# antrea-io/theia

Measured on AMD Instinct MI355X. Metric: flow-records/sec, higher is better.
Workload: dtype u64 (aggregates) + f64 (detectors)

## Files before the change

theia_amd/_capi.py:

```python
import ctypes as C
import os

from . import build as _build

u64, i64, i32, u32, f64, f32 = C.c_uint64, C.c_int64, C.c_int32, C.c_uint32, C.c_double, C.c_float

TAD_ABI_VERSION = 13
TAD_KEY_SKIP = (1 << 64) - 1
TAD_OK = 0
TAD_ERR_INVALID_ARGUMENT, TAD_ERR_NO_DEVICE, TAD_ERR_OUT_OF_MEMORY, TAD_ERR_HIP = -1, -2, -3, -4
TAD_ERR_KEY_RANGE, TAD_ERR_GRID_TOO_LARGE, TAD_ERR_BUSY = -5, -6, -7
TAD_ALGO = {"EWMA": 0, "ARIMA": 1, "DBSCAN": 2, "DROP": 3}
TAD_AGG = {"": 0, None: 0, "None": 0, "pod": 1, "svc": 2, "external": 3}
TAD_OP = {"auto": 0, "max": 1, "sum": 2}
TAD_MEM_HOST, TAD_MEM_DEVICE = 0, 1
TAD_FLAG_EMIT_ALL_POINTS = 1
TAD_FLAG_KEY_U32, TAD_FLAG_TIME_U32 = 2, 4
TAD_KEY_SKIP32 = (1 << 32) - 1
TAD_FEATURE_NARROW_COLUMNS = 1
TAD_FEATURE_STREAM_DBSCAN = 2
TAD_STATE_HISTORY = 1


class Plan(C.Structure):
    _fields_ = [("stage0", i32), ("partition_pass", i32), ("histogram", i32), ("sparse", i32), ("sparse_classes", i32),
                ("ewma_emit", i32), ("ewma_emit_rows", u32), ("reserved0", i32), ("tile_cells", i32), ("sparse_sort", i32), ("reserved1", i32)]


PLAN_VALUES = {
    "stage0": {"auto": 0, "v1": 1, "v2": 2}, "partition_pass": {"auto": 0, "sort": 1, "wc": 2, "wc_sectors": 3}, "histogram": {"auto": 0, "exact": 1, "sampled": 2},
    "sparse": {"auto": 0, "never": 1, "always": 2}, "sparse_classes": {"auto": 0, "always": 1}, "ewma_emit": {"auto": 0, "staged": 0, "lane": 1}, "tile_cells": {"auto": 0, "wide": 1},
    "sparse_sort": {"auto": 0, "lsd": 1, "partition": 2},
}


def make_plan(**kw):
    p = Plan()
    for name, v in kw.items():
        if name not in dict((f[0], 1) for f in Plan._fields_):
            raise ValueError("unknown tad_plan field %r" % name)
        if isinstance(v, str):
            v = PLAN_VALUES[name][v]
        setattr(p, name, int(v))
    return p


class KeyColumns(C.Structure):
    _fields_ = [("n_rows", u64), ("n_cols", i32), ("cols_a", C.POINTER(C.c_void_p)), ("keep_a", C.c_void_p),
                ("cols_b", C.POINTER(C.c_void_p)), ("keep_b", C.c_void_p), ("memory", C.c_int)]


class StringColumn(C.Structure):
    _fields_ = [("n_rows", u64), ("offsets", C.c_void_p), ("offset_bits", i32), ("data", C.c_void_p), ("data_bytes", u64),
                ("validity", C.c_void_p), ("validity_offset", u64), ("memory", C.c_int)]


class EngineOpts(C.Structure):
    _fields_ = [("device", i32), ("stream", C.c_void_p), ("workspace_limit", u64), ("plan", Plan), ("max_jobs_in_flight", i32), ("reserved", i32)]


class Job(C.Structure):
    _fields_ = [("algo", C.c_int), ("agg_flow", C.c_int), ("value_op", C.c_int),
                ("start_time", i64), ("end_time", i64), ("ewma_alpha", f64), ("dbscan_eps", f64),
                ("dbscan_min_samples", i32), ("arima_maxiter", i32), ("drop_nsigma", f64), ("drop_min_samples", i32),
# ... 108 lines not shown
```

theia_amd/csrc/tad_capi.cpp:

```cpp
#include "tad_engine.h"

using namespace tad;
using namespace tadh;

namespace tadh {

int ensure_rcp_table(JobCtx *e, uint64_t T) {
  const uint64_t want = T + 2;
  if (want <= e->rcp_n) return TAD_OK;
  uint64_t cap = want < 1024 ? 1024 : want + want / 4;
  int rc = ensure(e, e->rcp_table, cap * sizeof(double));
  if (rc != TAD_OK) return rc;
  std::vector<double> h(cap);
  h[0] = 0.0;
  for (uint64_t i = 1; i < cap; ++i) h[i] = 1.0 / (double)i;
  HIP_TRY(e, hipMemcpyAsync(e->rcp_table.p, h.data(), cap * sizeof(double), hipMemcpyHostToDevice, e->stream));
  HIP_TRY(e, hipStreamSynchronize(e->stream));
  e->rcp_n = cap;
  return TAD_OK;
}

int ensure_key_buffers(JobCtx *e, uint64_t K) {
  int rc;
  const uint64_t k = K ? K : 1;
  if ((rc = ensure(e, e->sigma, k * sizeof(double))) != TAD_OK) return rc;
  if ((rc = ensure(e, e->n_pts, k * sizeof(uint32_t))) != TAD_OK) return rc;
  if ((rc = ensure(e, e->n_anom, k * sizeof(uint32_t))) != TAD_OK) return rc;
  if ((rc = ensure(e, e->off, (k + 1) * sizeof(unsigned long long))) != TAD_OK) return rc;
  if ((rc = ensure(e, e->scan_scratch, scan_scratch_elems(k) * sizeof(unsigned long long))) != TAD_OK) return rc;
  if ((rc = ensure(e, e->key_mean, k * sizeof(double))) != TAD_OK) return rc;
  if ((rc = ensure(e, e->key_m2, k * sizeof(double))) != TAD_OK) return rc;
  if ((rc = ensure(e, e->counters, kTailBytes)) != TAD_OK) return rc;
  return TAD_OK;
}

}

namespace {

int detect_and_count(JobCtx *e, Grid g, JobParams &jp, DevCounters *ctr, uint64_t *rows, bool stats_done = false) {
  hipStream_t s = e->stream;
  int rc;
  if ((rc = ensure_key_buffers(e, g.K)) != TAD_OK) return rc;
  if ((rc = ensure_rcp_table(e, g.T)) != TAD_OK) return rc;
  double *sigma = static_cast<double *>(e->sigma.p);
  uint32_t *n_pts = static_cast<uint32_t *>(e->n_pts.p);
  uint32_t *n_anom = static_cast<uint32_t *>(e->n_anom.p);
  unsigned long long *off = static_cast<unsigned long long *>(e->off.p);

  const bool ewma = jp.algo == TAD_ALGO_EWMA;
  const bool drop = jp.algo == TAD_ALGO_DROP;
  const bool db_fused = jp.algo == TAD_ALGO_DBSCAN && !jp.all_points && !stats_done && dbscan_uses_list(g);
  jp.lazy_sigma = db_fused;
  if (drop) {
    if ((rc = ensure(e, e->calc, (g.K * g.T ? g.K * g.T : 1) * sizeof(double))) != TAD_OK) return rc;
    launch_drop(s, g, jp.drop_nsigma, jp.drop_min_samples, static_cast<double *>(e->calc.p), sigma, n_pts,
                static_cast<double *>(e->key_mean.p), static_cast<double *>(e->key_m2.p), ctr);
  } else if (!stats_done && !db_fused)
    launch_key_sigma(s, g, jp.alpha, ewma && !jp.all_points, static_cast<const double *>(e->rcp_table.p), sigma, n_pts, n_anom, ctr, static_cast<double *>(e->key_mean.p),
                     static_cast<double *>(e->key_m2.p));
  if (jp.algo == TAD_ALGO_DBSCAN) {
    if ((rc = ensure(e, e->aux, dbscan_scratch_bytes(g))) != TAD_OK) return rc;
    if (dbscan_uses_list(g)) {
      DbscanStats dst{nullptr, nullptr, nullptr, nullptr};
      if (db_fused) dst = DbscanStats{n_pts, n_anom, static_cast<double *>(e->key_mean.p), static_cast<double *>(e->key_m2.p)};
      if (launch_dbscan(s, g, jp.eps, jp.min_samples, e->aux.p, dst, jp.settled && db_fused) != 0)
        return fail(e, TAD_ERR_HIP, "DBSCAN launch failed");
    } else {
      return fail(e, TAD_ERR_GRID_TOO_LARGE, "DBSCAN: series of %llu buckets are not supported", (unsigned long long)g.T);
    }
  } else if (jp.algo == TAD_ALGO_ARIMA) {
    if ((rc = ensure(e, e->calc, g.K * g.T * sizeof(double))) != TAD_OK) return rc;
    const size_t wsb = arima_workspace_bytes(g);
    if ((rc = ensure(e, e->aux, wsb)) != TAD_OK) return rc;
    const bool held = e->hold && e->hold->held;
    if (held) e->hold->release();
    const unsigned int *yielded_dev = nullptr;
    if (launch_arima(s, g, sigma, n_pts, jp.maxiter, static_cast<double *>(e->calc.p), ctr, e->aux.p, wsb, e->eng->pause_dev, &yielded_dev) != 0)
      return fail(e, TAD_ERR_HIP, "ARIMA launch failed");
    while (yielded_dev != nullptr && e->eng->pause_dev != nullptr) {
      unsigned int y = 0;
      HIP_TRY(e, hipMemcpyAsync(&y, yielded_dev, 4, hipMemcpyDeviceToHost, s));
      HIP_TRY(e, hipStreamSynchronize(s));
      if (y == 0) break;
      const auto t0 = std::chrono::steady_clock::now();
      while (__atomic_load_n(&e->eng->pause_count, __ATOMIC_ACQUIRE) != 0 && std::chrono::steady_clock::now() - t0 < std::chrono::milliseconds(2))
        std::this_thread::sleep_for(std::chrono::microseconds(50));
      const uint32_t grace = __atomic_load_n(&e->eng->pause_count, __ATOMIC_ACQUIRE) != 0 ? 24u : 0u;
      if (launch_arima_fit(s, g, sigma, n_pts, jp.maxiter, static_cast<double *>(e->calc.p), ctr, e->aux.p, e->eng->pause_dev, &yielded_dev, grace) != 0)
        return fail(e, TAD_ERR_HIP, "ARIMA launch failed");
      e->arima_relaunches++;
    }
    if (held) e->hold->acquire();
  }
  const uint32_t *cnt = n_anom;
  if (jp.all_points && jp.algo != TAD_ALGO_ARIMA && !drop) cnt = n_pts;
  else if (db_fused) {}
  else if (!ewma || jp.all_points) launch_count_flags(s, g, jp.all_points, n_anom);
  launch_scan_moments(s, cnt, off, g.K, static_cast<unsigned long long *>(e->scan_scratch.p), dev_total(e), n_pts,
                      static_cast<const double *>(e->key_mean.p), static_cast<const double *>(e->key_m2.p), dev_moments(e), db_fused ? ctr : nullptr);
  HIP_TRY(e, hipMemcpyAsync(e->tail_host, e->counters.p, kTailBytes, hipMemcpyDeviceToHost, s));
  HIP_TRY(e, hipStreamSynchronize(s));
  HIP_TRY(e, hipGetLastError());
  *rows = *e->total_host;
  return TAD_OK;
}

}

namespace tadh {

void emit_rows(JobCtx *e, Grid g, Lattice L, const JobParams &jp, OutRows out, uint64_t rows) {
  const int kind = jp.algo == TAD_ALGO_EWMA ? 0 : (jp.algo == TAD_ALGO_ARIMA ? 1 : (jp.algo == TAD_ALGO_DROP ? 3 : (jp.lazy_sigma ? 4 : 2)));
  if (kind == 4 && !jp.all_points &&
      launch_emit_dbscan_list(e->stream, g, L, e->aux.p, static_cast<const uint32_t *>(e->n_anom.p), static_cast<const unsigned long long *>(e->off.p), out))
    return;
  launch_emit(e->stream, g, L, kind, jp.all_points, jp.alpha, static_cast<const double *>(e->sigma.p),
              static_cast<const uint32_t *>(e->n_pts.p), static_cast<const double *>(kind == 3 ? e->key_mean.p : e->calc.p),
              static_cast<const unsigned long long *>(e->off.p), out, rows, e->plan.ewma_emit, e->plan.ewma_emit_rows);
}

}

namespace {

int make_result(JobCtx *e, uint64_t rows, bool with_anomaly, tad_mem out_memory, ResultPriv **out, OutRows *dev_rows,
                ResultBlock *dev_block) {
  ResultPriv *rp = new (std::nothrow) ResultPriv();
  if (!rp) return fail(e, TAD_ERR_OUT_OF_MEMORY, "out of host memory");
  memset(rp, 0, sizeof *rp);
  const size_t bytes = result_bytes(rows, with_anomaly);
  int rc = alloc_device_block(e, bytes, dev_block);
  if (rc != TAD_OK) { delete rp; return rc; }
  carve(dev_block->base, rows, with_anomaly, dev_rows);
  rp->pub.n_rows = rows;
  rp->pub.memory = out_memory;
  *out = rp;
  return TAD_OK;
}

int finish_result(JobCtx *e, ResultPriv *rp, uint64_t rows, bool with_anomaly, ResultBlock dev_block, OutRows dev_rows) {
  if (rp->pub.memory == TAD_MEM_DEVICE) {
    rp->block = dev_block.base;
    rp->block_cap = dev_block.cap;
    rp->pub.key_id = reinterpret_cast<uint64_t *>(dev_rows.key_id);
    rp->pub.flow_end_s = reinterpret_cast<int64_t *>(dev_rows.flow_end_s);
    rp->pub.throughput = dev_rows.throughput;
    rp->pub.algo_calc = dev_rows.algo_calc;
    rp->pub.stddev = dev_rows.stddev;
    rp->pub.anomaly = dev_rows.anomaly;
    return TAD_OK;
  }
// ... 1219 lines not shown
```

theia_amd/csrc/tad_engine.cpp:

```cpp
#include "tad_engine.h"

using namespace tad;
using namespace tadh;

namespace tadh {

thread_local std::string g_static_err;

bool plan_ok(const tad_plan &p) {
  return p.stage0 >= 0 && p.stage0 <= 2 && p.partition_pass >= 0 && p.partition_pass <= 3 && p.histogram >= 0 && p.histogram <= 2 && p.sparse >= 0 &&
         p.sparse <= 2 && p.sparse_classes >= 0 && p.sparse_classes <= 1 && p.ewma_emit >= 0 && p.ewma_emit <= 1 && p.ewma_emit_rows <= 4096 && p.tile_cells >= 0 && p.tile_cells <= 1 && p.sparse_sort >= 0 && p.sparse_sort <= 2 && p.reserved0 == 0 && p.reserved1 == 0;
}

int vfail(tad_engine *e, int code, const char *fmt, va_list ap) {
  char buf[512];
  vsnprintf(buf, sizeof buf, fmt, ap);
  if (e) {
    std::lock_guard<std::mutex> lk(e->err_mu);
    e->err = buf;
  } else {
    g_static_err = buf;
  }
  return code;
}
int fail(tad_engine *e, int code, const char *fmt, ...) {
  va_list ap;
  va_start(ap, fmt);
  const int rc = vfail(e, code, fmt, ap);
  va_end(ap);
  return rc;
}
int fail(JobCtx *c, int code, const char *fmt, ...) {
  va_list ap;
  va_start(ap, fmt);
  const int rc = vfail(c ? c->eng : nullptr, code, fmt, ap);
  va_end(ap);
  return rc;
}
int fail(std::nullptr_t, int code, const char *fmt, ...) {
  va_list ap;
  va_start(ap, fmt);
  const int rc = vfail(nullptr, code, fmt, ap);
  va_end(ap);
  return rc;
// ... 394 lines not shown
```

theia_amd/csrc/tad_engine.h:

```cpp
#ifndef THEIA_TAD_ENGINE_H
#define THEIA_TAD_ENGINE_H

#include <atomic>
#include <chrono>
#include <condition_variable>
#include <cstdarg>
#include <cstdio>
#include <cstdlib>
#include <cstring>
#include <mutex>
#include <new>
#include <string>
#include <thread>
#include <vector>

#include "tad_internal.h"

struct DevBuf {
  void *p = nullptr;
  size_t cap = 0;
};

struct FreeBlock {
  void *p;
// ... 20 lines not shown
  int pause_count = 0;
  int *pause_dev = nullptr;
  hipStream_t signal_stream = nullptr;
  std::mutex pool_mu;
  std::vector<FreeBlock> free_blocks;
};

struct PauseHold;
struct JobCtx {
  tad_engine *eng = nullptr;
  PauseHold *hold = nullptr;
  int index = 0;
  bool busy = false;
  int device = 0;
  hipStream_t stream = nullptr;
  hipStream_t stream_normal = nullptr, stream_low = nullptr;
  bool own_streams = false;
  uint64_t ws_limit = 0;
  tad_plan plan{};
  std::atomic<int32_t> done{0}, total{0};
  char id[64] = {};
  DevBuf grid_val, grid_flag, sigma, n_pts, n_anom, off, scan_scratch, calc, counters, meta, aux, key_mean, key_m2;
  DevBuf in_key, in_key2, in_te, in_ts, in_val;
  DevBuf rcp_table;
  uint64_t rcp_n = 0;
  DevBuf binhist, part_total, part_start, part_offs32, recs, ovf, slices;
  DevBuf sp_comp_a, sp_comp_b, sp_val_a, sp_val_b, sp_temp, sp_first, sp_times;
  DevBuf sp_cls;
  DevBuf hs_key, hs_t, hs_val, hs_sorted, hs_noise, hs_cnt, hs_row, hs_koff, hs_kcnt;
  int arima_relaunches = 0;
  bool sp_by_partition = false;
  DevBuf part_fin;
  DevBuf ovf_keys;
  hipEvent_t ev[8] = {};
  tad::MetaPartial *meta_host = nullptr;
  unsigned char *tail_host = nullptr;
  tad::DevCounters *ctr_host = nullptr;
  unsigned long long *total_host = nullptr;
  tad::Moments *moments_host = nullptr;
  struct Learnt {
    bool valid = false;
    uint64_t n = 0, K = 0;
    bool has2 = false;
    int algo = 0, op = 0;
    bool exact_hist = false;
    uint32_t exact_uses = 0, exact_backoff = 8;
    bool wide_tiles = false;
  } learnt;
};

struct tad_state {
  uint64_t K = 0;
  void *block[2] = {nullptr, nullptr};
  int cur = 0;
  bool history = false;
  unsigned long long *hist_off[2] = {nullptr, nullptr};
  unsigned long long *hist_val[2] = {nullptr, nullptr};
  uint64_t hist_cap[2] = {0, 0};
  uint64_t hist_len[2] = {0, 0};
  mutable std::mutex mu;
};

struct PauseHold {
  tad_engine *eng;
  bool held = false;
  explicit PauseHold(tad_engine *e) : eng(e) {}
// ... 18 lines not shown
using namespace tad;

extern thread_local std::string g_static_err;

constexpr size_t kTailCtr = 0, kTailTotal = 64, kTailOvfCount = 72, kTailHistLen = 80, kTailMoments = 128;
constexpr size_t kTailBytes = kTailMoments + sizeof(Moments) * kMomentBlocks;
inline unsigned long long *dev_total(JobCtx *e) { return reinterpret_cast<unsigned long long *>(static_cast<unsigned char *>(e->counters.p) + kTailTotal); }
inline unsigned long long *dev_ovf_count(JobCtx *e) { return reinterpret_cast<unsigned long long *>(static_cast<unsigned char *>(e->counters.p) + kTailOvfCount); }
inline Moments *dev_moments(JobCtx *e) { return reinterpret_cast<Moments *>(static_cast<unsigned char *>(e->counters.p) + kTailMoments); }

constexpr int kMetaBlocks = 2048;
constexpr int kSampleBlockShift = 7;
constexpr int kDefaultJobsInFlight = 4;
constexpr int kMaxJobsInFlight = 16;
constexpr uint32_t kOverflowCap = 1u << 20;

bool plan_ok(const tad_plan &p);
int fail(tad_engine *e, int code, const char *fmt, ...);
int fail(JobCtx *c, int code, const char *fmt, ...);
int fail(std::nullptr_t, int code, const char *fmt, ...);

#define HIP_TRY(e, call)                                                                         \
  do {                                                                                           \
    hipError_t err__ = (call);                                                                   \
    if (err__ != hipSuccess)                                                                     \
      return fail((e), err__ == hipErrorOutOfMemory ? TAD_ERR_OUT_OF_MEMORY : TAD_ERR_HIP,       \
                  "%s failed: %s (%s:%d)", #call, hipGetErrorString(err__), __FILE__, __LINE__); \
  } while (0)


template <typename F> void for_each_buf(JobCtx *c, F f) {
  DevBuf *bufs[] = {&c->grid_val, &c->grid_flag, &c->sigma, &c->n_pts, &c->n_anom, &c->off, &c->scan_scratch, &c->calc, &c->counters, &c->meta, &c->aux,
                    &c->key_mean, &c->key_m2, &c->rcp_table, &c->binhist, &c->part_total, &c->part_start, &c->part_offs32, &c->recs, &c->ovf, &c->slices,
                    &c->sp_comp_a, &c->sp_comp_b, &c->sp_val_a, &c->sp_val_b, &c->sp_temp, &c->sp_first, &c->sp_times, &c->sp_cls, &c->part_fin, &c->ovf_keys,
                    &c->in_key, &c->in_key2, &c->in_te, &c->in_ts, &c->in_val,
                    &c->hs_key, &c->hs_t, &c->hs_val, &c->hs_sorted, &c->hs_noise, &c->hs_cnt, &c->hs_row, &c->hs_koff, &c->hs_kcnt};
  for (DevBuf *b : bufs) f(*b);
}

void drop_buffers(JobCtx *c);
void trim_idle(tad_engine *eng, JobCtx *self);
int ensure(JobCtx *e, DevBuf &b, size_t bytes);
void preload_code_objects();
JobCtx *ctx_create(tad_engine *eng, bool first);
void ctx_destroy(JobCtx *c);

struct Lease {
  tad_engine *eng;
  JobCtx *c = nullptr;
  Lease(tad_engine *eng_, const char *id = nullptr, bool low_priority = false) : eng(eng_) {
    std::unique_lock<std::mutex> lk(eng->mu);
    for (;;) {
      for (JobCtx *x : eng->ctxs)
        if (!x->busy) { c = x; break; }
      if (c) break;
      if ((int)eng->ctxs.size() + eng->creating < eng->max_ctx) {
        ++eng->creating;
        lk.unlock();
        hipSetDevice(eng->device);
        JobCtx *n = ctx_create(eng, false);
        lk.lock();
        --eng->creating;
        if (n) { n->index = (int)eng->ctxs.size(); eng->ctxs.push_back(n); c = n; break; }
        if (eng->ctxs.empty()) return;
      }
      eng->cv.wait(lk);
    }
// ... 28 lines not shown
Lattice make_lattice(int64_t t0, int64_t step, uint64_t nb);
uint64_t host_gcd(uint64_t a, uint64_t b);

struct ResultBlock {
  void *base = nullptr;
  size_t cap = 0;
};

size_t result_bytes(uint64_t rows, bool with_anomaly);
void carve(void *base, uint64_t rows, bool with_anomaly, OutRows *o);
int alloc_device_block(JobCtx *e, size_t bytes, ResultBlock *rb);

struct ResultPriv {
  tad_result pub;
  void *block;
  size_t block_cap;
};

struct PointsPriv {
  tad_points pub;
  void *block;
  size_t block_cap;
};

struct JobParams {
  tad_algo algo;
  double alpha, eps;
  int min_samples, maxiter;
  double drop_nsigma;
  int drop_min_samples;
  bool all_points;
  bool lazy_sigma = false;
  bool settled = false;
};

int ensure_rcp_table(JobCtx *e, uint64_t T);
int ensure_key_buffers(JobCtx *e, uint64_t K);
void emit_rows(JobCtx *e, Grid g, Lattice L, const JobParams &jp, OutRows out, uint64_t rows = 0);

}

#endif
```

theia_amd/csrc/tad_internal.h:

```cpp
#pragma once
#include <hip/hip_runtime.h>
#include <stdint.h>
#include <type_traits>

#include "tad.h"

namespace tad {

struct Lattice {
  int64_t t0;
  int64_t step;
  uint64_t nb;
  uint64_t magic;
  int mode;
};

struct Grid {
  unsigned long long *val;
  uint8_t *flag;
  uint64_t K;
  uint64_t T;
  const long long *times;
};

// ... 144 lines not shown
  uint32_t f0, f1, f2;
  unsigned long long v0, v1, v2;
  load(0, f0, v0);
  load(1, f1, v1);
  for (uint64_t c = 0; c < nblk; ++c) {
    load(c + 2, f2, v2);
    const uint64_t t0 = c * 64;
    const double x0 = (double)v0;
    const unsigned long long present = __ballot((f0 & FLAG_PRESENT) != 0);
    block(c);
    int ord = 0;
    for (unsigned long long m = present; m; m &= m - 1, ++ord) {
      const int u = __ffsll((long long)m) - 1;
      step(t0 + (uint64_t)u, (uint8_t)readlane_u32(f0, u), readlane_f64(x0, u), ord);
    }
    f0 = f1; v0 = v1;
    f1 = f2; v1 = v2;
  }
}

__device__ __forceinline__ Moments chan_merge(Moments a, Moments b) {
  if (b.n == 0.0) return a;
  if (a.n == 0.0) return b;
  Moments r;
  r.n = a.n + b.n;
  const double d = b.mean - a.mean;
  r.mean = a.mean + d * (b.n / r.n);
  r.m2 = a.m2 + b.m2 + d * d * (a.n * b.n / r.n);
  return r;
}

#endif

void launch_key_sigma(hipStream_t s, Grid g, double alpha, bool ewma_count, const double *rcp, double *sigma,
                      uint32_t *n_pts, uint32_t *n_anom, DevCounters *ctr, double *key_mean, double *key_m2);
static constexpr int kMomentBlocks = 128;
void launch_moments(hipStream_t s, uint64_t K, const uint32_t *n_pts, const double *key_mean,
                    const double *key_m2, Moments *partials, DevCounters *ctr = nullptr);
void launch_count_flags(hipStream_t s, Grid g, bool all_points, uint32_t *n_anom);
void launch_scan(hipStream_t s, const uint32_t *cnt, unsigned long long *off, uint64_t K,
                 unsigned long long *scratch, unsigned long long *total_copy = nullptr);
size_t scan_scratch_elems(uint64_t K);
void launch_scan_moments(hipStream_t s, const uint32_t *cnt, unsigned long long *off, uint64_t K, unsigned long long *scratch,
                         unsigned long long *total_copy, const uint32_t *n_pts, const double *key_mean, const double *key_m2, Moments *partials,
                         DevCounters *ctr);
void launch_emit(hipStream_t s, Grid g, Lattice lat, int kind, bool all_points, double alpha,
                 const double *sigma, const uint32_t *n_pts, const double *calc,
                 const unsigned long long *off, OutRows out, uint64_t rows_hint = 0,
                 int ewma_emit = 0, uint32_t ewma_emit_rows = 0);
void launch_emit_points(hipStream_t s, Grid g, Lattice lat, const unsigned long long *off, unsigned long long *out_key,
                        long long *out_t, unsigned long long *out_val);
struct StreamState {
  uint32_t *n;
  double *avg, *m2, *ewma;
  long long *last_t;
  unsigned char *seen;
};
void launch_stream(hipStream_t s, Grid g, Lattice lat, double alpha, bool all_points, bool emit, StreamState cur, StreamState next,
                   uint32_t *n_anom, const unsigned long long *off, OutRows out, DevCounters *ctr);
void launch_stream_points(hipStream_t s, const unsigned long long *comp, const unsigned long long *val, const unsigned long long *poff, uint64_t K,
                          int64_t t0, double alpha, bool all_points, bool emit, StreamState cur, StreamState next, uint32_t *n_anom,
                          const unsigned long long *off, OutRows out, DevCounters *ctr);
void launch_hist_decode(hipStream_t s, const unsigned long long *comp, uint64_t P, int64_t t0, unsigned long long *nk, long long *nt);
void launch_hist_sort(hipStream_t s, const unsigned long long *nv, const unsigned long long *poff, uint64_t K, unsigned long long *ns,
                      uint32_t *long_list, unsigned int *long_count);
uint64_t hist_merge_chunks_bound(uint64_t K, uint64_t total_len);
void launch_hist_merge(hipStream_t s, uint64_t K, const unsigned long long *hoff_old, const unsigned long long *hval_old, const unsigned long long *poff,
                       const unsigned long long *ns, unsigned long long *hoff_new, unsigned long long *hval_new, uint32_t *chunks,
                       unsigned long long *coff, unsigned long long *scan_scratch, uint64_t chunks_bound);
void launch_hist_verdict(hipStream_t s, const unsigned long long *nk, const unsigned long long *nv, const unsigned long long *P_dev, uint64_t P_cap,
                         const unsigned long long *hoff, const unsigned long long *h, double eps, int min_samples, bool all_points, uint8_t *noise,
                         uint32_t *cnt);
void launch_hist_emit(hipStream_t s, const unsigned long long *nk, const long long *nt, const unsigned long long *nv, const unsigned long long *P_dev,
                      uint64_t P_cap, const uint8_t *noise, const uint32_t *cnt, const unsigned long long *row, StreamState next, bool all_points,
                      OutRows out);
void launch_ewma_values(hipStream_t s, Grid g, double alpha, double *calc);

struct DbscanStats {
  uint32_t *n_pts, *n_anom;
  double *key_mean, *key_m2;
};
struct SettleArgs {
// ... 154 lines not shown
```

theia_amd/csrc/tad_kernels.hip:

```cpp
#include <cstdlib>

#include "tad_internal.h"

namespace tad {

static constexpr int kBlock = 256;

__device__ __forceinline__ uint64_t gcd_u64(uint64_t a, uint64_t b) {
  if (a == 0) return b;
  if (b == 0) return a;
  if (((a | b) >> 32) == 0) {
    uint32_t x = (uint32_t)a, y = (uint32_t)b;
    while (y) { uint32_t r = x % y; x = y; y = r; }
    return x;
  }
  while (b) { uint64_t r = a % b; a = b; b = r; }
  return a;
}

__device__ __forceinline__ uint64_t absdiff_i64(int64_t a, int64_t b) {
  return a >= b ? (uint64_t)a - (uint64_t)b : (uint64_t)b - (uint64_t)a;
}

struct MetaAcc {
  int64_t tmin, tmax, tref;
  uint64_t g, used;
};

__device__ __forceinline__ MetaAcc meta_merge(MetaAcc a, const MetaAcc &b) {
  if (b.used == 0) return a;
  if (a.used == 0) return b;
  a.tmin = b.tmin < a.tmin ? b.tmin : a.tmin;
// ... 145 lines not shown
  }
  unsigned long long u = used;
  for (int d = 32; d >= 1; d >>= 1) {
    u += __shfl_down(u, d);
    err |= __shfl_down(err, d);
  }
  if ((threadIdx.x & 63) == 0) {
    if (u) atomicAdd(&ctr->rows_used, u);
    if (err) atomicOr(&ctr->err, err);
  }
}

void launch_scatter(hipStream_t s, const uint64_t *key, const uint64_t *key2, const int64_t *t_end,
                    const int64_t *t_start, const uint64_t *value, uint64_t n, RowFilter f,
                    Lattice lat, Grid g, bool op_max, DevCounters *ctr, int cw) {
  if (n == 0) return;
  auto aligned16 = [](const void *p) { return p == nullptr || (reinterpret_cast<uintptr_t>(p) & 15) == 0; };
  const bool vec = aligned16(key) && aligned16(key2) && aligned16(t_end) && aligned16(value) && n >= 2;
  const uint64_t work = vec ? (n >> 1) : n;
  int blocks = (int)((work + kBlock - 1) / kBlock);
  if (blocks > 256 * 16) blocks = 256 * 16;
  if (blocks < 1) blocks = 1;
  with_widths(cw, [&](auto k32, auto t32) {
#define TAD_LAUNCH_SCATTER(OPMAX, VEC) \
  hipLaunchKernelGGL((k_scatter<OPMAX, VEC, k32(), t32()>), dim3(blocks), dim3(kBlock), 0, s, key, key2, t_end, t_start, value, n, f, lat, g, ctr)
    if (op_max) { if (vec) TAD_LAUNCH_SCATTER(true, true); else TAD_LAUNCH_SCATTER(true, false); }
    else        { if (vec) TAD_LAUNCH_SCATTER(false, true); else TAD_LAUNCH_SCATTER(false, false); }
#undef TAD_LAUNCH_SCATTER
  });
}

static constexpr int kUnroll = 16;

template <bool EWMA_COUNT, bool RCP_LDS, bool COOP = false>
__global__ __launch_bounds__(kBlock) void k_key_sigma(Grid g, double alpha, const double *__restrict__ rcp_g, double *__restrict__ sigma,
                                                      uint32_t *__restrict__ n_pts,
                                                      uint32_t *__restrict__ n_anom, DevCounters *ctr,
                                                      double *__restrict__ key_mean, double *__restrict__ key_m2) {
  const uint64_t gtid = (uint64_t)blockIdx.x * kBlock + threadIdx.x;
  const uint64_t k = COOP ? gtid >> 6 : gtid;
  const bool writer = !COOP || (threadIdx.x & 63) == 0;
  extern __shared__ __attribute__((aligned(16))) unsigned char smem_rcp[];
  const double *rcp = rcp_g;
  if (RCP_LDS) {
    double *l = reinterpret_cast<double *>(smem_rcp);
    for (uint64_t i = threadIdx.x; i <= g.T; i += kBlock) l[i] = rcp_g[i];
    __syncthreads();
    rcp = l;
  }
  unsigned long long my_pts = 0;
  unsigned my_key = 0;
  if (k < g.K) {
    double cnt = 0.0, avg = 0.0, m2 = 0.0;
    uint32_t n = 0;
    auto sigma_step = [&](uint64_t, uint8_t fl, unsigned long long raw) {
      if (fl & FLAG_PRESENT) {
        const double x = (double)raw;
        cnt = cnt + 1.0;
        n++;
        const double d = x - avg;
        const double dn = RCP_LDS ? div_by_count(d, cnt, rcp[n]) : d / cnt;
        avg = avg + dn;
        m2 = m2 + d * (d - dn);
      }
    };
    if (COOP) {
      double rl = 0.0;
      walk_series_coop(g, k,
                       [&](uint64_t) { rl = 1.0 / (double)(n + 1u + (threadIdx.x & 63u)); },
                       [&](uint64_t, uint8_t, double x, int ord) {
                         cnt = cnt + 1.0;
                         n++;
                         const double d = x - avg;
                         const double dn = div_by_count(d, cnt, readlane_f64(rl, ord));
                         avg = avg + dn;
                         m2 = m2 + d * (d - dn);
                       });
    } else {
      walk_series(g, k, sigma_step);
    }
    const bool has_sigma = n >= 2;
    const double sg = has_sigma ? sqrt(m2 / (cnt - 1.0)) : 0.0;
    if (writer) {
      sigma[k] = sg;
      n_pts[k] = n;
      if (key_mean != nullptr) { key_mean[k] = avg; key_m2[k] = m2; }
      my_pts = n;
      my_key = n > 0;
    }
    if (EWMA_COUNT) {
      uint32_t a = 0;
      if (has_sigma) {
        const double one_minus = 1.0 - alpha;
        double e = 0.0;
        auto ewma_step = [&](uint64_t, uint8_t fl, unsigned long long raw) {
          if (fl & FLAG_PRESENT) {
            const double x = (double)raw;
            e = one_minus * e + alpha * x;
            a += fabs(x - e) > sg ? 1u : 0u;
          }
        };
        if (COOP) walk_series_coop(g, k, [](uint64_t) {}, [&](uint64_t, uint8_t, double x, int) {
                    e = one_minus * e + alpha * x;
                    a += fabs(x - e) > sg ? 1u : 0u;
                  });
        else walk_series(g, k, ewma_step);
      }
      if (writer) n_anom[k] = a;
    }
  }
  for (int d = 32; d >= 1; d >>= 1) {
    my_pts += __shfl_down(my_pts, d);
    my_key += __shfl_down(my_key, d);
  }
  if ((threadIdx.x & 63) == 0 && my_key) {
    atomicAdd(&ctr->n_points, my_pts);
    atomicAdd(&ctr->n_keys, (unsigned long long)my_key);
  }
}

void launch_key_sigma(hipStream_t s, Grid g, double alpha, bool ewma_count, const double *rcp, double *sigma,
                      uint32_t *n_pts, uint32_t *n_anom, DevCounters *ctr, double *key_mean, double *key_m2) {
  if (g.K == 0) return;
  const size_t lds = (size_t)(g.T + 1) * 8;
  const bool in_lds = lds <= 32768;
  if (coop_shape(g)) {
    const int cblocks = (int)((g.K * 64 + kBlock - 1) / kBlock);
#define TAD_KSC(EC, RL) hipLaunchKernelGGL((k_key_sigma<EC, RL, true>), dim3(cblocks), dim3(kBlock), RL ? lds : 0, s, g, alpha, rcp, sigma, n_pts, n_anom, ctr, key_mean, key_m2)
    if (ewma_count) { if (in_lds) TAD_KSC(true, true); else TAD_KSC(true, false); }
    else { if (in_lds) TAD_KSC(false, true); else TAD_KSC(false, false); }
#undef TAD_KSC
    return;
  }
  const int blocks = (int)((g.K + kBlock - 1) / kBlock);
#define TAD_KS(EC, RL) hipLaunchKernelGGL((k_key_sigma<EC, RL>), dim3(blocks), dim3(kBlock), RL ? lds : 0, s, g, alpha, rcp, sigma, n_pts, n_anom, ctr, key_mean, key_m2)
  if (ewma_count) { if (in_lds) TAD_KS(true, true); else TAD_KS(true, false); }
  else { if (in_lds) TAD_KS(false, true); else TAD_KS(false, false); }
#undef TAD_KS
}


struct MomentsArgs {
  uint64_t K;
  const uint32_t *n_pts;
  const double *key_mean, *key_m2;
  Moments *partials;
  DevCounters *ctr;
};

__device__ __forceinline__ void moments_block(uint32_t mb, uint64_t K, const uint32_t *__restrict__ n_pts,
                                              const double *__restrict__ key_mean,
                                              const double *__restrict__ key_m2,
                                              Moments *__restrict__ partials, DevCounters *ctr) {
  Moments acc{0.0, 0.0, 0.0};
  unsigned long long pts = 0, keys = 0;
  const uint64_t stride = (uint64_t)kMomentBlocks * kBlock;
  constexpr int kMU = 8;
  for (uint64_t k = (uint64_t)mb * kBlock + threadIdx.x; k < K; k += stride * kMU) {
    uint32_t n[kMU];
    double mean[kMU], m2[kMU];
#pragma unroll
    for (int u = 0; u < kMU; ++u) {
      const uint64_t ku = k + (uint64_t)u * stride;
      const bool in = ku < K;
      n[u] = in ? n_pts[ku] : 0u;
      mean[u] = in ? key_mean[ku] : 0.0;
      m2[u] = in ? key_m2[ku] : 0.0;
    }
// ... 258 lines not shown
          const ulonglong2 kk = make_ulonglong2(k, k);
          reinterpret_cast<ulonglong2 *>(out.key_id + pos)[0] = kk;
          reinterpret_cast<ulonglong2 *>(out.key_id + pos)[1] = kk;
          reinterpret_cast<longlong2 *>(out.flow_end_s + pos)[0] = make_longlong2(bt[0], bt[1]);
          reinterpret_cast<longlong2 *>(out.flow_end_s + pos)[1] = make_longlong2(bt[2], bt[3]);
          reinterpret_cast<double2 *>(out.throughput + pos)[0] = make_double2(bx[0], bx[1]);
          reinterpret_cast<double2 *>(out.throughput + pos)[1] = make_double2(bx[2], bx[3]);
          reinterpret_cast<double2 *>(out.algo_calc + pos)[0] = make_double2(ba[0], ba[1]);
          reinterpret_cast<double2 *>(out.algo_calc + pos)[1] = make_double2(ba[2], ba[3]);
          if (!LAZY) {
            const double2 ss = make_double2(sg, sg);
            reinterpret_cast<double2 *>(out.stddev + pos)[0] = ss;
            reinterpret_cast<double2 *>(out.stddev + pos)[1] = ss;
          }
          if (ALL) *reinterpret_cast<uint32_t *>(out.anomaly + pos) = (uint32_t)bv[0] | ((uint32_t)bv[1] << 8) | ((uint32_t)bv[2] << 16) | ((uint32_t)bv[3] << 24);
          pos += 4;
          nb = 0;
        }
      }
    }
  };
  if (COOP) walk_series_coop(g, k, [](uint64_t) {}, [&](uint64_t t, uint8_t fl, double x, int) { point(t, fl, x); });
  else walk_series(g, k, [&](uint64_t t, uint8_t fl, unsigned long long raw) { if (fl & FLAG_PRESENT) point(t, fl, (double)raw); });
#pragma unroll
  for (int i = 0; i < 3; ++i)
    if (i < nb) write_row(pos + i, bt[i], bx[i], ba[i], ALL && bv[i] != 0);
  if (LAZY) {
    sg = has_sigma ? sqrt(s_m2 / (s_cnt - 1.0)) : 0.0;
    if (COOP) { for (unsigned long long at = first + (threadIdx.x & 63); at < end; at += 64) out.stddev[at] = sg; }
    else { for (unsigned long long at = first; at < end; ++at) out.stddev[at] = sg; }
  }
}

static constexpr int kStageMarkTBits = 26;
__global__ __launch_bounds__(64) void k_emit_staged(Grid g, Lattice L, double alpha, const double *__restrict__ sigma,
                                                    const uint32_t *__restrict__ n_pts,
                                                    const unsigned long long *__restrict__ off, OutRows out, uint32_t cap) {
  extern __shared__ __attribute__((aligned(16))) unsigned char smem_stage[];
  double *s_e = reinterpret_cast<double *>(smem_stage);
  double *s_sg = s_e + cap;
  uint32_t *s_m = reinterpret_cast<uint32_t *>(s_sg + 64);
  const uint32_t lane = threadIdx.x;
  const uint64_t k0 = (uint64_t)blockIdx.x * 64;
  const uint64_t k = k0 + lane;
  const uint64_t kend = k0 + 64 < g.K ? k0 + 64 : g.K;
  const unsigned long long base = off[k0];
  const unsigned long long total = off[kend] - base;
  if (total == 0) return;
  const bool live = k < g.K;
  unsigned long long pos = live ? off[k] - base : 0;
  const unsigned long long end = live ? off[k + 1] - base : 0;
  const double sg = live ? sigma[k] : 0.0;
  s_sg[lane] = sg;
  if (pos != end) {
    const double one_minus = 1.0 - alpha;
    double e = 0.0;
    walk_series(g, k, [&](uint64_t t, uint8_t fl, unsigned long long raw) {
      if (!(fl & FLAG_PRESENT)) return;
      const double x = (double)raw;
      e = one_minus * e + alpha * x;
      if (fabs(x - e) > sg && pos < end) {
        if (pos < cap) {
          s_e[pos] = e;
          s_m[pos] = (lane << kStageMarkTBits) | (uint32_t)t;
        } else {
          const unsigned long long at = base + pos;
          out.key_id[at] = k;
          out.flow_end_s[at] = g.times != nullptr ? g.times[t * g.K + k] : (long long)(L.t0 + (int64_t)t * L.step);
          out.throughput[at] = x;
          out.algo_calc[at] = e;
          out.stddev[at] = sg;
        }
        pos++;
      }
    });
  }
  __syncthreads();
  const unsigned long long staged = total < cap ? total : cap;
  for (unsigned long long r = lane; r < staged; r += 64) {
    const uint32_t m = s_m[r];
    const uint32_t ln = m >> kStageMarkTBits;
    const uint64_t t = m & ((1u << kStageMarkTBits) - 1u);
    const uint64_t cell = t * g.K + (k0 + ln);
    const unsigned long long at = base + r;
    out.key_id[at] = k0 + ln;
    out.flow_end_s[at] = g.times != nullptr ? g.times[cell] : (long long)(L.t0 + (int64_t)t * L.step);
    out.throughput[at] = (double)g.val[cell];
    out.algo_calc[at] = s_e[r];
    out.stddev[at] = s_sg[ln];
  }
}

static uint32_t emit_stage_rows(uint64_t K, uint64_t rows_hint, int ewma_emit, uint32_t ewma_emit_rows) {
  if (ewma_emit == 1) return 0;
  uint64_t cap = 1536;
  if (rows_hint != 0) {
    const uint64_t mean = (rows_hint * 64 + K - 1) / K;
    cap = mean + mean / 8 + 128;
  }
  if (ewma_emit_rows != 0) cap = ewma_emit_rows;
  cap = (cap + 63) & ~63ull;
  if (cap < 64) cap = 64;
  if (cap > 4096) cap = 4096;
  return (uint32_t)cap;
}

void launch_emit(hipStream_t s, Grid g, Lattice lat, int kind, bool all_points, double alpha,
                 const double *sigma, const uint32_t *n_pts, const double *calc,
                 const unsigned long long *off, OutRows out, uint64_t rows_hint, int ewma_emit, uint32_t ewma_emit_rows) {
  if (g.K == 0) return;
  if (coop_shape(g)) {
    const int cblocks = (int)((g.K * 64 + kBlock - 1) / kBlock);
#define TAD_LAUNCH_EMIT_C(KIND, ALL) \
  hipLaunchKernelGGL((k_emit<KIND, ALL, true>), dim3(cblocks), dim3(kBlock), 0, s, g, lat, alpha, sigma, n_pts, calc, off, out)
    if (all_points) {
      if (kind == 0) TAD_LAUNCH_EMIT_C(0, true); else if (kind == 1) TAD_LAUNCH_EMIT_C(1, true); else if (kind == 3) TAD_LAUNCH_EMIT_C(3, true); else TAD_LAUNCH_EMIT_C(2, true);
    } else {
      if (kind == 0) TAD_LAUNCH_EMIT_C(0, false); else if (kind == 1) TAD_LAUNCH_EMIT_C(1, false); else if (kind == 3) TAD_LAUNCH_EMIT_C(3, false);
      else if (kind == 4) TAD_LAUNCH_EMIT_C(4, false); else TAD_LAUNCH_EMIT_C(2, false);
    }
#undef TAD_LAUNCH_EMIT_C
    return;
  }
  if (kind == 0 && !all_points && g.T < (1ull << kStageMarkTBits)) {
    if (const uint32_t cap = emit_stage_rows(g.K, rows_hint, ewma_emit, ewma_emit_rows)) {
      const unsigned blocks64 = (unsigned)((g.K + 63) / 64);
      hipLaunchKernelGGL(k_emit_staged, dim3(blocks64), dim3(64), (size_t)cap * 12 + 64 * 8, s, g, lat, alpha, sigma, n_pts, off, out, cap);
      return;
    }
  }
  const int blocks = (int)((g.K + kBlock - 1) / kBlock);
#define TAD_LAUNCH_EMIT(KIND, ALL) \
  hipLaunchKernelGGL((k_emit<KIND, ALL>), dim3(blocks), dim3(kBlock), 0, s, g, lat, alpha, sigma, n_pts, calc, off, out)
  if (all_points) {
    if (kind == 0) TAD_LAUNCH_EMIT(0, true); else if (kind == 1) TAD_LAUNCH_EMIT(1, true); else if (kind == 3) TAD_LAUNCH_EMIT(3, true); else TAD_LAUNCH_EMIT(2, true);
  } else {
    if (kind == 0) TAD_LAUNCH_EMIT(0, false); else if (kind == 1) TAD_LAUNCH_EMIT(1, false); else if (kind == 3) TAD_LAUNCH_EMIT(3, false);
    else if (kind == 4) TAD_LAUNCH_EMIT(4, false); else TAD_LAUNCH_EMIT(2, false);
  }
#undef TAD_LAUNCH_EMIT
}

__global__ __launch_bounds__(kBlock) void k_emit_points(Grid g, Lattice L, const unsigned long long *__restrict__ off,
                                                        unsigned long long *__restrict__ out_key, long long *__restrict__ out_t,
                                                        unsigned long long *__restrict__ out_val) {
  const uint64_t k = (uint64_t)blockIdx.x * kBlock + threadIdx.x;
  if (k >= g.K) return;
  unsigned long long pos = off[k];
  const unsigned long long end = off[k + 1];
  auto step = [&](uint64_t t, uint8_t fl, unsigned long long raw) {
    if ((fl & FLAG_PRESENT) && pos < end) {
      out_key[pos] = k;
      out_t[pos] = g.times != nullptr ? g.times[t * g.K + k] : (long long)(L.t0 + (int64_t)t * L.step);
      out_val[pos] = raw;
      pos++;
    }
  };
  uint64_t t = 0;
  for (; t + kUnroll <= g.T && pos < end; t += kUnroll) {
    uint8_t fl[kUnroll];
// ... 190 lines not shown
```

Before: 78.01 billion.

## Stage EWMA anomaly rows during sigma pass so emit copies instead of recomputing

```diff
diff --git a/theia_amd/_capi.py b/theia_amd/_capi.py
--- a/theia_amd/_capi.py
+++ b/theia_amd/_capi.py
@@ -29,7 +29,7 @@
 
 PLAN_VALUES = {
     "stage0": {"auto": 0, "v1": 1, "v2": 2}, "partition_pass": {"auto": 0, "sort": 1, "wc": 2, "wc_sectors": 3}, "histogram": {"auto": 0, "exact": 1, "sampled": 2},
-    "sparse": {"auto": 0, "never": 1, "always": 2}, "sparse_classes": {"auto": 0, "always": 1}, "ewma_emit": {"auto": 0, "staged": 0, "lane": 1}, "tile_cells": {"auto": 0, "wide": 1},
+    "sparse": {"auto": 0, "never": 1, "always": 2}, "sparse_classes": {"auto": 0, "always": 1}, "ewma_emit": {"auto": 0, "staged": 0, "copy": 0, "lane": 1, "walk": 2}, "tile_cells": {"auto": 0, "wide": 1},
     "sparse_sort": {"auto": 0, "lsd": 1, "partition": 2},
 }
 
diff --git a/theia_amd/csrc/tad_capi.cpp b/theia_amd/csrc/tad_capi.cpp
--- a/theia_amd/csrc/tad_capi.cpp
+++ b/theia_amd/csrc/tad_capi.cpp
@@ -56,9 +56,17 @@
     if ((rc = ensure(e, e->calc, (g.K * g.T ? g.K * g.T : 1) * sizeof(double))) != TAD_OK) return rc;
     launch_drop(s, g, jp.drop_nsigma, jp.drop_min_samples, static_cast<double *>(e->calc.p), sigma, n_pts,
                 static_cast<double *>(e->key_mean.p), static_cast<double *>(e->key_m2.p), ctr);
-  } else if (!stats_done && !db_fused)
+  } else if (!stats_done && !db_fused) {
+    jp.ewma_stage = EwmaStage{nullptr, nullptr, nullptr, 0};
+    if (ewma && !jp.all_points) {
+      if (const uint32_t cap = ewma_stage_rows(g, e->plan.ewma_emit, e->plan.ewma_emit_rows)) {
+        if ((rc = ensure(e, e->ewma_stage, ewma_stage_bytes(g.K, cap))) != TAD_OK) return rc;
+        jp.ewma_stage = ewma_stage_carve(e->ewma_stage.p, g.K, cap);
+      }
+    }
     launch_key_sigma(s, g, jp.alpha, ewma && !jp.all_points, static_cast<const double *>(e->rcp_table.p), sigma, n_pts, n_anom, ctr, static_cast<double *>(e->key_mean.p),
-                     static_cast<double *>(e->key_m2.p));
+                     static_cast<double *>(e->key_m2.p), jp.ewma_stage);
+  }
   if (jp.algo == TAD_ALGO_DBSCAN) {
     if ((rc = ensure(e, e->aux, dbscan_scratch_bytes(g))) != TAD_OK) return rc;
     if (dbscan_uses_list(g)) {
@@ -117,7 +125,8 @@
     return;
   launch_emit(e->stream, g, L, kind, jp.all_points, jp.alpha, static_cast<const double *>(e->sigma.p),
               static_cast<const uint32_t *>(e->n_pts.p), static_cast<const double *>(kind == 3 ? e->key_mean.p : e->calc.p),
-              static_cast<const unsigned long long *>(e->off.p), out, rows, e->plan.ewma_emit, e->plan.ewma_emit_rows);
+              static_cast<const unsigned long long *>(e->off.p), out, rows, e->plan.ewma_emit, e->plan.ewma_emit_rows,
+              kind == 0 && !jp.all_points && jp.ewma_stage.cap != 0 ? &jp.ewma_stage : nullptr);
 }
 
 }
diff --git a/theia_amd/csrc/tad_engine.cpp b/theia_amd/csrc/tad_engine.cpp
--- a/theia_amd/csrc/tad_engine.cpp
+++ b/theia_amd/csrc/tad_engine.cpp
@@ -9,7 +9,7 @@
 
 bool plan_ok(const tad_plan &p) {
   return p.stage0 >= 0 && p.stage0 <= 2 && p.partition_pass >= 0 && p.partition_pass <= 3 && p.histogram >= 0 && p.histogram <= 2 && p.sparse >= 0 &&
-         p.sparse <= 2 && p.sparse_classes >= 0 && p.sparse_classes <= 1 && p.ewma_emit >= 0 && p.ewma_emit <= 1 && p.ewma_emit_rows <= 4096 && p.tile_cells >= 0 && p.tile_cells <= 1 && p.sparse_sort >= 0 && p.sparse_sort <= 2 && p.reserved0 == 0 && p.reserved1 == 0;
+         p.sparse <= 2 && p.sparse_classes >= 0 && p.sparse_classes <= 1 && p.ewma_emit >= 0 && p.ewma_emit <= 2 && p.ewma_emit_rows <= 4096 && p.tile_cells >= 0 && p.tile_cells <= 1 && p.sparse_sort >= 0 && p.sparse_sort <= 2 && p.reserved0 == 0 && p.reserved1 == 0;
 }
 
 int vfail(tad_engine *e, int code, const char *fmt, va_list ap) {
diff --git a/theia_amd/csrc/tad_engine.h b/theia_amd/csrc/tad_engine.h
--- a/theia_amd/csrc/tad_engine.h
+++ b/theia_amd/csrc/tad_engine.h
@@ -76,6 +76,7 @@
   bool sp_by_partition = false;
   DevBuf part_fin;
   DevBuf ovf_keys;
+  DevBuf ewma_stage;
   hipEvent_t ev[8] = {};
   tad::MetaPartial *meta_host = nullptr;
   unsigned char *tail_host = nullptr;
@@ -160,7 +161,7 @@
 template <typename F> void for_each_buf(JobCtx *c, F f) {
   DevBuf *bufs[] = {&c->grid_val, &c->grid_flag, &c->sigma, &c->n_pts, &c->n_anom, &c->off, &c->scan_scratch, &c->calc, &c->counters, &c->meta, &c->aux,
                     &c->key_mean, &c->key_m2, &c->rcp_table, &c->binhist, &c->part_total, &c->part_start, &c->part_offs32, &c->recs, &c->ovf, &c->slices,
-                    &c->sp_comp_a, &c->sp_comp_b, &c->sp_val_a, &c->sp_val_b, &c->sp_temp, &c->sp_first, &c->sp_times, &c->sp_cls, &c->part_fin, &c->ovf_keys,
+                    &c->sp_comp_a, &c->sp_comp_b, &c->sp_val_a, &c->sp_val_b, &c->sp_temp, &c->sp_first, &c->sp_times, &c->sp_cls, &c->part_fin, &c->ovf_keys, &c->ewma_stage,
                     &c->in_key, &c->in_key2, &c->in_te, &c->in_ts, &c->in_val,
                     &c->hs_key, &c->hs_t, &c->hs_val, &c->hs_sorted, &c->hs_noise, &c->hs_cnt, &c->hs_row, &c->hs_koff, &c->hs_kcnt};
   for (DevBuf *b : bufs) f(*b);
@@ -255,6 +256,7 @@
   bool all_points;
   bool lazy_sigma = false;
   bool settled = false;
+  tad::EwmaStage ewma_stage{nullptr, nullptr, nullptr, 0};
 };
 
 int ensure_rcp_table(JobCtx *e, uint64_t T);
diff --git a/theia_amd/csrc/tad_internal.h b/theia_amd/csrc/tad_internal.h
--- a/theia_amd/csrc/tad_internal.h
+++ b/theia_amd/csrc/tad_internal.h
@@ -200,8 +200,16 @@
 
 #endif
 
+struct EwmaStage {
+  double *e;
+  uint32_t *m, *n;
+  uint32_t cap;
+};
+uint32_t ewma_stage_rows(const Grid &g, int ewma_emit, uint32_t ewma_emit_rows);
+size_t ewma_stage_bytes(uint64_t K, uint32_t cap);
+EwmaStage ewma_stage_carve(void *p, uint64_t K, uint32_t cap);
 void launch_key_sigma(hipStream_t s, Grid g, double alpha, bool ewma_count, const double *rcp, double *sigma,
-                      uint32_t *n_pts, uint32_t *n_anom, DevCounters *ctr, double *key_mean, double *key_m2);
+                      uint32_t *n_pts, uint32_t *n_anom, DevCounters *ctr, double *key_mean, double *key_m2, EwmaStage st = EwmaStage{nullptr, nullptr, nullptr, 0});
 static constexpr int kMomentBlocks = 128;
 void launch_moments(hipStream_t s, uint64_t K, const uint32_t *n_pts, const double *key_mean,
                     const double *key_m2, Moments *partials, DevCounters *ctr = nullptr);
@@ -215,7 +223,8 @@
 void launch_emit(hipStream_t s, Grid g, Lattice lat, int kind, bool all_points, double alpha,
                  const double *sigma, const uint32_t *n_pts, const double *calc,
                  const unsigned long long *off, OutRows out, uint64_t rows_hint = 0,
-                 int ewma_emit = 0, uint32_t ewma_emit_rows = 0);
+                 int ewma_emit = 0, uint32_t ewma_emit_rows = 0,
+                 const EwmaStage *stage = nullptr);
 void launch_emit_points(hipStream_t s, Grid g, Lattice lat, const unsigned long long *off, unsigned long long *out_key,
                         long long *out_t, unsigned long long *out_val);
 struct StreamState {
diff --git a/theia_amd/csrc/tad_kernels.hip b/theia_amd/csrc/tad_kernels.hip
--- a/theia_amd/csrc/tad_kernels.hip
+++ b/theia_amd/csrc/tad_kernels.hip
@@ -1,3 +1,4 @@
+#include <algorithm>
 #include <cstdlib>
 
 #include "tad_internal.h"
@@ -209,22 +210,74 @@
 
 static constexpr int kUnroll = 16;
 
-template <bool EWMA_COUNT, bool RCP_LDS, bool COOP = false>
+static constexpr int kStageMarkTBits = 26;
+static constexpr int kStageRankShift = 13;
+static constexpr uint32_t kStageRankMask = ((1u << (kStageMarkTBits - kStageRankShift)) - 1u) << kStageRankShift;
+static constexpr uint32_t kStageOverflow = 0xFFFFFFFFu;
+static size_t ewma_stage_lds_bytes(uint32_t cap) { return (size_t)cap * 14 + 64 * 4; }
+
+__device__ __forceinline__ void ewma_stage_wave(uint32_t a, const EwmaStage &st, const double *s_e, const uint32_t *s_m, uint16_t *s_idx,
+                                                uint32_t *s_base) {
+  const uint32_t lane = threadIdx.x & 63u;
+  __syncthreads();
+  uint32_t incl = a;
+  for (int d = 1; d < 64; d <<= 1) {
+    const uint32_t y = __shfl_up(incl, d);
+    if (lane >= (uint32_t)d) incl += y;
+  }
+  const uint32_t total = __shfl(incl, 63);
+  const uint64_t w = blockIdx.x;
+  if (lane == 0) st.n[w] = total <= st.cap ? total : kStageOverflow;
+  if (total > st.cap) return;
+  s_base[lane] = incl - a;
+  __syncthreads();
+  constexpr int kU = 4;
+  for (uint32_t r0 = lane; r0 < total; r0 += 64 * kU) {
+    uint32_t m[kU];
+#pragma unroll
+    for (int u = 0; u < kU; ++u) m[u] = r0 + 64 * u < total ? s_m[r0 + 64 * u] : 0u;
+#pragma unroll
+    for (int u = 0; u < kU; ++u)
+      if (r0 + 64 * u < total) s_idx[s_base[m[u] >> kStageMarkTBits] + ((m[u] & kStageRankMask) >> kStageRankShift)] = (uint16_t)(r0 + 64 * u);
+  }
+  __syncthreads();
+  double *ge = st.e + w * st.cap;
+  uint32_t *gm = st.m + w * st.cap;
+  for (uint32_t r0 = lane; r0 < total; r0 += 64 * kU) {
+    uint32_t i[kU];
+#pragma unroll
+    for (int u = 0; u < kU; ++u) i[u] = r0 + 64 * u < total ? s_idx[r0 + 64 * u] : 0u;
+#pragma unroll
+    for (int u = 0; u < kU; ++u)
+      if (r0 + 64 * u < total) {
+        ge[r0 + 64 * u] = s_e[i[u]];
+        gm[r0 + 64 * u] = s_m[i[u]] & ~kStageRankMask;
+      }
+  }
+}
+
+template <bool EWMA_COUNT, bool RCP_LDS, bool COOP = false, bool STAGE = false>
 __global__ __launch_bounds__(kBlock) void k_key_sigma(Grid g, double alpha, const double *__restrict__ rcp_g, double *__restrict__ sigma,
                                                       uint32_t *__restrict__ n_pts,
                                                       uint32_t *__restrict__ n_anom, DevCounters *ctr,
-                                                      double *__restrict__ key_mean, double *__restrict__ key_m2) {
-  const uint64_t gtid = (uint64_t)blockIdx.x * kBlock + threadIdx.x;
+                                                      double *__restrict__ key_mean, double *__restrict__ key_m2, EwmaStage st) {
+  constexpr int BS = STAGE ? 64 : kBlock;
+  const uint64_t gtid = (uint64_t)blockIdx.x * BS + threadIdx.x;
   const uint64_t k = COOP ? gtid >> 6 : gtid;
   const bool writer = !COOP || (threadIdx.x & 63) == 0;
   extern __shared__ __attribute__((aligned(16))) unsigned char smem_rcp[];
   const double *rcp = rcp_g;
   if (RCP_LDS) {
     double *l = reinterpret_cast<double *>(smem_rcp);
-    for (uint64_t i = threadIdx.x; i <= g.T; i += kBlock) l[i] = rcp_g[i];
+    for (uint64_t i = threadIdx.x; i <= g.T; i += BS) l[i] = rcp_g[i];
     __syncthreads();
     rcp = l;
   }
+  double *s_e = reinterpret_cast<double *>(smem_rcp);
+  uint32_t *s_m = reinterpret_cast<uint32_t *>(s_e + (STAGE ? st.cap : 0));
+  uint16_t *s_idx = reinterpret_cast<uint16_t *>(s_m + (STAGE ? st.cap : 0));
+  uint32_t *s_base = reinterpret_cast<uint32_t *>(s_idx + (STAGE ? st.cap : 0));
+  uint32_t a = 0;
   unsigned long long my_pts = 0;
   unsigned my_key = 0;
   if (k < g.K) {
@@ -266,12 +319,28 @@
       my_key = n > 0;
     }
     if (EWMA_COUNT) {
-      uint32_t a = 0;
+      if (STAGE) __builtin_amdgcn_wave_barrier();
       if (has_sigma) {
         const double one_minus = 1.0 - alpha;
         double e = 0.0;
-        auto ewma_step = [&](uint64_t, uint8_t fl, unsigned long long raw) {
-          if (fl & FLAG_PRESENT) {
+        uint32_t cursor = 0;
+        auto ewma_step = [&](uint64_t t, uint8_t fl, unsigned long long raw) {
+          if constexpr (STAGE) {
+            bool hit = false;
+            if (fl & FLAG_PRESENT) {
+              const double x = (double)raw;
+              e = one_minus * e + alpha * x;
+              hit = fabs(x - e) > sg;
+            }
+            const unsigned long long b = __ballot(hit);
+            const uint32_t slot = cursor + __builtin_amdgcn_mbcnt_hi((uint32_t)(b >> 32), __builtin_amdgcn_mbcnt_lo((uint32_t)b, 0u));
+            if (hit && slot < st.cap) {
+              s_e[slot] = e;
+              s_m[slot] = ((threadIdx.x & 63u) << kStageMarkTBits) | (a << kStageRankShift) | (uint32_t)t;
+            }
+            cursor += (uint32_t)__popcll(b);
+            a += hit ? 1u : 0u;
+          } else if (fl & FLAG_PRESENT) {
             const double x = (double)raw;
             e = one_minus * e + alpha * x;
             a += fabs(x - e) > sg ? 1u : 0u;
@@ -286,6 +355,7 @@
       if (writer) n_anom[k] = a;
     }
   }
+  if constexpr (STAGE) ewma_stage_wave(a, st, s_e, s_m, s_idx, s_base);
   for (int d = 32; d >= 1; d >>= 1) {
     my_pts += __shfl_down(my_pts, d);
     my_key += __shfl_down(my_key, d);
@@ -297,20 +367,28 @@
 }
 
 void launch_key_sigma(hipStream_t s, Grid g, double alpha, bool ewma_count, const double *rcp, double *sigma,
-                      uint32_t *n_pts, uint32_t *n_anom, DevCounters *ctr, double *key_mean, double *key_m2) {
+                      uint32_t *n_pts, uint32_t *n_anom, DevCounters *ctr, double *key_mean, double *key_m2, EwmaStage st) {
   if (g.K == 0) return;
   const size_t lds = (size_t)(g.T + 1) * 8;
   const bool in_lds = lds <= 32768;
+  if (ewma_count && st.cap != 0) {
+    const size_t slds = std::max(in_lds ? lds : (size_t)0, ewma_stage_lds_bytes(st.cap));
+    const unsigned blocks64 = (unsigned)((g.K + 63) / 64);
+#define TAD_KSS(RL) hipLaunchKernelGGL((k_key_sigma<true, RL, false, true>), dim3(blocks64), dim3(64), slds, s, g, alpha, rcp, sigma, n_pts, n_anom, ctr, key_mean, key_m2, st)
+    if (in_lds) TAD_KSS(true); else TAD_KSS(false);
+#undef TAD_KSS
+    return;
+  }
   if (coop_shape(g)) {
     const int cblocks = (int)((g.K * 64 + kBlock - 1) / kBlock);
-#define TAD_KSC(EC, RL) hipLaunchKernelGGL((k_key_sigma<EC, RL, true>), dim3(cblocks), dim3(kBlock), RL ? lds : 0, s, g, alpha, rcp, sigma, n_pts, n_anom, ctr, key_mean, key_m2)
+#define TAD_KSC(EC, RL) hipLaunchKernelGGL((k_key_sigma<EC, RL, true>), dim3(cblocks), dim3(kBlock), RL ? lds : 0, s, g, alpha, rcp, sigma, n_pts, n_anom, ctr, key_mean, key_m2, st)
     if (ewma_count) { if (in_lds) TAD_KSC(true, true); else TAD_KSC(true, false); }
     else { if (in_lds) TAD_KSC(false, true); else TAD_KSC(false, false); }
 #undef TAD_KSC
     return;
   }
   const int blocks = (int)((g.K + kBlock - 1) / kBlock);
-#define TAD_KS(EC, RL) hipLaunchKernelGGL((k_key_sigma<EC, RL>), dim3(blocks), dim3(kBlock), RL ? lds : 0, s, g, alpha, rcp, sigma, n_pts, n_anom, ctr, key_mean, key_m2)
+#define TAD_KS(EC, RL) hipLaunchKernelGGL((k_key_sigma<EC, RL>), dim3(blocks), dim3(kBlock), RL ? lds : 0, s, g, alpha, rcp, sigma, n_pts, n_anom, ctr, key_mean, key_m2, st)
   if (ewma_count) { if (in_lds) TAD_KS(true, true); else TAD_KS(true, false); }
   else { if (in_lds) TAD_KS(false, true); else TAD_KS(false, false); }
 #undef TAD_KS
@@ -635,10 +713,8 @@
   }
 }
 
-static constexpr int kStageMarkTBits = 26;
-__global__ __launch_bounds__(64) void k_emit_staged(Grid g, Lattice L, double alpha, const double *__restrict__ sigma,
-                                                    const uint32_t *__restrict__ n_pts,
-                                                    const unsigned long long *__restrict__ off, OutRows out, uint32_t cap) {
+__device__ __forceinline__ void emit_staged_wave(Grid g, Lattice L, double alpha, const double *__restrict__ sigma,
+                                                 const unsigned long long *__restrict__ off, OutRows out, uint32_t cap) {
   extern __shared__ __attribute__((aligned(16))) unsigned char smem_stage[];
   double *s_e = reinterpret_cast<double *>(smem_stage);
   double *s_sg = s_e + cap;
@@ -694,6 +770,66 @@
   }
 }
 
+__global__ __launch_bounds__(64) void k_emit_staged(Grid g, Lattice L, double alpha, const double *__restrict__ sigma,
+                                                    const uint32_t *__restrict__ n_pts,
+                                                    const unsigned long long *__restrict__ off, OutRows out, uint32_t cap) {
+  emit_staged_wave(g, L, alpha, sigma, off, out, cap);
+}
+
+__global__ __launch_bounds__(64) void k_emit_copy(Grid g, Lattice L, double alpha, const double *__restrict__ sigma,
+                                                  const unsigned long long *__restrict__ off, OutRows out, uint32_t cap, EwmaStage st) {
+  extern __shared__ __attribute__((aligned(16))) unsigned char smem_stage[];
+  const uint32_t lane = threadIdx.x;
+  const uint64_t w = blockIdx.x;
+  const uint64_t k0 = w * 64;
+  const uint64_t kend = k0 + 64 < g.K ? k0 + 64 : g.K;
+  const unsigned long long base = off[k0];
+  const unsigned long long total = off[kend] - base;
+  if (total == 0) return;
+  if (st.n[w] != total) {
+    emit_staged_wave(g, L, alpha, sigma, off, out, cap);
+    return;
+  }
+  double *s_sg = reinterpret_cast<double *>(smem_stage);
+  s_sg[lane] = k0 + lane < g.K ? sigma[k0 + lane] : 0.0;
+  __syncthreads();
+  const double *__restrict__ ge = st.e + w * st.cap;
+  const uint32_t *__restrict__ gm = st.m + w * st.cap;
+  constexpr int kU = 8;
+  for (unsigned long long r0 = lane; r0 < total; r0 += 64 * kU) {
+    double e[kU];
+    uint32_t m[kU];
+    unsigned long long v[kU];
+    long long ts[kU];
+#pragma unroll
+    for (int u = 0; u < kU; ++u) {
+      const unsigned long long r = r0 + 64 * u;
+      e[u] = r < total ? ge[r] : 0.0;
+      m[u] = r < total ? gm[r] : 0u;
+    }
+#pragma unroll
+    for (int u = 0; u < kU; ++u) {
+      const uint64_t t = m[u] & ((1u << kStageMarkTBits) - 1u);
+      const uint64_t cell = t * g.K + (k0 + (m[u] >> kStageMarkTBits));
+      const bool in = r0 + 64 * u < total;
+      v[u] = in ? g.val[cell] : 0ull;
+      ts[u] = !in ? 0ll : (g.times != nullptr ? g.times[cell] : (long long)(L.t0 + (int64_t)t * L.step));
+    }
+#pragma unroll
+    for (int u = 0; u < kU; ++u) {
+      const unsigned long long r = r0 + 64 * u;
+      if (r < total) {
+        const unsigned long long at = base + r;
+        out.key_id[at] = k0 + (m[u] >> kStageMarkTBits);
+        out.flow_end_s[at] = ts[u];
+        out.throughput[at] = (double)v[u];
+        out.algo_calc[at] = e[u];
+        out.stddev[at] = s_sg[m[u] >> kStageMarkTBits];
+      }
+    }
+  }
+}
+
 static uint32_t emit_stage_rows(uint64_t K, uint64_t rows_hint, int ewma_emit, uint32_t ewma_emit_rows) {
   if (ewma_emit == 1) return 0;
   uint64_t cap = 1536;
@@ -708,9 +844,26 @@
   return (uint32_t)cap;
 }
 
+uint32_t ewma_stage_rows(const Grid &g, int ewma_emit, uint32_t ewma_emit_rows) {
+  if (g.K == 0 || ewma_emit != 0 || coop_shape(g) || g.T > (1ull << kStageRankShift)) return 0;
+  return emit_stage_rows(g.K, 0, ewma_emit, ewma_emit_rows);
+}
+
+size_t ewma_stage_bytes(uint64_t K, uint32_t cap) {
+  const uint64_t w = (K + 63) / 64;
+  return (size_t)w * cap * 12 + (size_t)w * 4;
+}
+
+EwmaStage ewma_stage_carve(void *p, uint64_t K, uint32_t cap) {
+  const uint64_t w = (K + 63) / 64;
+  double *e = static_cast<double *>(p);
+  uint32_t *m = reinterpret_cast<uint32_t *>(e + w * cap);
+  return EwmaStage{e, m, m + w * cap, cap};
+}
+
 void launch_emit(hipStream_t s, Grid g, Lattice lat, int kind, bool all_points, double alpha,
                  const double *sigma, const uint32_t *n_pts, const double *calc,
-                 const unsigned long long *off, OutRows out, uint64_t rows_hint, int ewma_emit, uint32_t ewma_emit_rows) {
+                 const unsigned long long *off, OutRows out, uint64_t rows_hint, int ewma_emit, uint32_t ewma_emit_rows, const EwmaStage *stage) {
   if (g.K == 0) return;
   if (coop_shape(g)) {
     const int cblocks = (int)((g.K * 64 + kBlock - 1) / kBlock);
@@ -728,7 +881,10 @@
   if (kind == 0 && !all_points && g.T < (1ull << kStageMarkTBits)) {
     if (const uint32_t cap = emit_stage_rows(g.K, rows_hint, ewma_emit, ewma_emit_rows)) {
       const unsigned blocks64 = (unsigned)((g.K + 63) / 64);
-      hipLaunchKernelGGL(k_emit_staged, dim3(blocks64), dim3(64), (size_t)cap * 12 + 64 * 8, s, g, lat, alpha, sigma, n_pts, off, out, cap);
+      if (stage != nullptr && stage->cap != 0)
+        hipLaunchKernelGGL(k_emit_copy, dim3(blocks64), dim3(64), (size_t)cap * 12 + 64 * 8, s, g, lat, alpha, sigma, off, out, cap, *stage);
+      else
+        hipLaunchKernelGGL(k_emit_staged, dim3(blocks64), dim3(64), (size_t)cap * 12 + 64 * 8, s, g, lat, alpha, sigma, n_pts, off, out, cap);
       return;
     }
   }
```

New measurement: 78.03 billion, median of 6. About the same (+0.0%).
